# pearl-robot-lab/2HandedAfforder

Hardware: AMD Instinct MI355X
Metric: affordance frames/sec/GPU @1024^2, 32-tok prompt; mask IoU vs ref (higher is better)
Workload: dtype bf16; 1 GPU; BASELINE.json configs[2]: 2HandedAfforder-7B, 64 x 1024x1024 uint8 NHWC frames/step/GPU, 32-token prompt (T=291), 8 forced answer tokens with [SEG], KV-cached greedy decode, random-init weights; CLIP + SAM preprocessing of the uint8 frames on the device inside the step; parallelism=frame-sharded replicas x1 (no collective), hip_streams=2, fp32_decoder_tail=True, fp32_residual_stream=off, neck_f32=False, sam_chunk=16, sam_waits_for_prefill=False, decode_chain=False

## Files before the change

2handedafforder_amd/csrc/gemm_f32.hip:

```cpp
#include "haff_common.h"

namespace {

constexpr int TM = 128, TN = 128, TK = 16, RS = 20;

struct GemmF32Args {
  const float* A; long lda;
  const float* W; long ldw;
  float* C; long ldc;
  const float* bias;
  const float* resid; long ldr;
  const int* row_map;
  int M, N, K;
  int act, swiglu;
  int nb_inner;
  long sAo, sAi, sWo, sWi, sCo, sCi;
};

__global__ __launch_bounds__(256) void gemm_f32_kernel(GemmF32Args p) {
  __shared__ __attribute__((aligned(16))) float sA[2][TM * RS];
  __shared__ __attribute__((aligned(16))) float sW[2][TN * RS];
  if (p.nb_inner > 0) {
    const int zo = blockIdx.y / p.nb_inner, zi = blockIdx.y - zo * p.nb_inner;
    p.A += zo * p.sAo + zi * p.sAi;
    p.W += zo * p.sWo + zi * p.sWi;
    p.C += zo * p.sCo + zi * p.sCi;
  }
  const int tid = threadIdx.x, lane = tid & 63, wave = tid >> 6;
  const int wm = wave & 1, wn = wave >> 1;
  const int fr = lane & 15, fg = lane >> 4;
  const int tiles_n = (p.N + TN - 1) / TN;
  const int tm = blockIdx.x / tiles_n, tn = blockIdx.x - tm * tiles_n;
  const int m0 = tm * TM, n0 = tn * TN;

  f32x4 acc[4][4];
#pragma unroll
  for (int i = 0; i < 4; ++i)
#pragma unroll
    for (int j = 0; j < 4; ++j) acc[i][j] = f32x4{0.f, 0.f, 0.f, 0.f};

  const int lrow = tid >> 2, lk = (tid & 3) * 4;
  const float* a0 = p.A + (long)min(m0 + lrow, p.M - 1) * p.lda + lk;
  const float* a1 = p.A + (long)min(m0 + lrow + 64, p.M - 1) * p.lda + lk;
  const float* w0 = p.W + (long)min(n0 + lrow, p.N - 1) * p.ldw + lk;
  const float* w1 = p.W + (long)min(n0 + lrow + 64, p.N - 1) * p.ldw + lk;
  const float4 z4 = make_float4(0.f, 0.f, 0.f, 0.f);
  float4 ra0, ra1, rw0, rw1;
  auto fetch = [&](int k0) {
    const bool ok = k0 + lk < p.K;
    ra0 = ok ? *reinterpret_cast<const float4*>(a0 + k0) : z4;
    ra1 = ok ? *reinterpret_cast<const float4*>(a1 + k0) : z4;
    rw0 = ok ? *reinterpret_cast<const float4*>(w0 + k0) : z4;
    rw1 = ok ? *reinterpret_cast<const float4*>(w1 + k0) : z4;
  };
  auto stash = [&](int buf) {
    *reinterpret_cast<float4*>(&sA[buf][lrow * RS + lk]) = ra0;
    *reinterpret_cast<float4*>(&sA[buf][(lrow + 64) * RS + lk]) = ra1;
    *reinterpret_cast<float4*>(&sW[buf][lrow * RS + lk]) = rw0;
    *reinterpret_cast<float4*>(&sW[buf][(lrow + 64) * RS + lk]) = rw1;
  };
  const int nk = (p.K + TK - 1) / TK;
  fetch(0);
  stash(0);
  __syncthreads();
  for (int kt = 0; kt < nk; ++kt) {
    const int buf = kt & 1;
// ... 137 lines not shown

template <int MR>
static void launch_f32_skinny(const GemmF32Args& p, hipStream_t s) {
  if (p.N >= 2048) hipLaunchKernelGGL((gemm_f32_skinny_kernel<MR, 4>), dim3((p.N + 3) / 4), dim3(256), 0, s, p);
  else if (p.N >= 512) hipLaunchKernelGGL((gemm_f32_skinny_kernel<MR, 2>), dim3((p.N + 1) / 2), dim3(256), 0, s, p);
  else hipLaunchKernelGGL((gemm_f32_skinny_kernel<MR, 1>), dim3(p.N), dim3(256), 0, s, p);
}

}

extern "C" int haff_gemm_f32(const float* A, long lda, const float* W, long ldw, float* C, long ldc,
                             const float* bias, const float* resid, long ldr, const int* row_map, int M, int N, int K,
                             int act, int swiglu, void* stream) {
  if (M <= 0 || N <= 0 || K <= 0 || (K & 3) || (lda & 3) || (ldw & 3)) return HAFF_ERR_BAD_ARG;
  if (swiglu && ((N & 31) || resid)) return HAFF_ERR_BAD_ARG;
  GemmF32Args p{A, lda, W, ldw, C, ldc, bias, resid, ldr, row_map, M, N, K, act, swiglu, 0, 0, 0, 0, 0, 0, 0};
  hipStream_t s = reinterpret_cast<hipStream_t>(stream);
  const bool al16 = ((reinterpret_cast<uintptr_t>(A) | reinterpret_cast<uintptr_t>(W)) & 15) == 0;
  if (!swiglu && al16 && (M <= 8 || (M <= 16 && (long)N * K <= (1L << 21)))) {
    if (M <= 1) launch_f32_skinny<1>(p, s);
    else if (M <= 4) launch_f32_skinny<4>(p, s);
    else if (M <= 8) launch_f32_skinny<8>(p, s);
    else launch_f32_skinny<16>(p, s);
    return haff_check_launch();
  }
  const int tiles = ((M + TM - 1) / TM) * ((N + TN - 1) / TN);
  hipLaunchKernelGGL(gemm_f32_kernel, dim3(tiles), dim3(256), 0, s, p);
  return haff_check_launch();
}

extern "C" int haff_gemm_f32_batched(const float* A, long lda, long sAo, long sAi, const float* W, long ldw, long sWo,
                                     long sWi, float* C, long ldc, long sCo, long sCi, int nb_outer, int nb_inner, int M,
                                     int N, int K, void* stream) {
  if (M <= 0 || N <= 0 || K <= 0 || nb_outer <= 0 || nb_inner <= 0) return HAFF_ERR_BAD_ARG;
  if ((K & 3) || (lda & 3) || (ldw & 3) || (sAo & 3) || (sAi & 3) || (sWo & 3) || (sWi & 3)) return HAFF_ERR_BAD_ARG;
  GemmF32Args p{A, lda, W, ldw, C, ldc, nullptr, nullptr, 0, nullptr, M, N, K, 0, 0, nb_inner, sAo, sAi, sWo, sWi, sCo, sCi};
  const int tiles = ((M + TM - 1) / TM) * ((N + TN - 1) / TN);
  hipLaunchKernelGGL(gemm_f32_kernel, dim3(tiles, nb_outer * nb_inner), dim3(256), 0, reinterpret_cast<hipStream_t>(stream), p);
  return haff_check_launch();
}
```

2handedafforder_amd/lib.py:

```python
import ctypes
import os
import subprocess

_HERE = os.path.dirname(os.path.abspath(__file__))
LIB_PATH = os.environ.get("HAFF_LIB_PATH") or os.path.join(_HERE, "lib", "libhaff_hip.so")
CSRC_DIR = os.path.join(_HERE, "csrc")

c_void_p, c_long, c_int, c_float = ctypes.c_void_p, ctypes.c_long, ctypes.c_int, ctypes.c_float

_PROTOS = {
    "haff_gemm_bf16": [c_void_p, c_long, c_void_p, c_long, c_void_p, c_long, c_void_p, c_void_p, c_long, c_void_p,
                       c_int, c_int, c_int, c_int, c_int, c_int, c_void_p],
    "haff_gemm_bf16_cfg": [c_void_p, c_long, c_void_p, c_long, c_void_p, c_long, c_void_p, c_void_p, c_long, c_void_p,
                           c_int, c_int, c_int, c_int, c_int, c_int, c_int, c_void_p],
    "haff_gemm_bf16_ws": [c_void_p, c_long, c_void_p, c_long, c_void_p, c_long, c_void_p, c_void_p, c_long, c_void_p,
                          c_int, c_int, c_int, c_int, c_int, c_int, c_void_p, c_long, c_void_p],
    "haff_gemm_bf16_rms": [c_void_p, c_long, c_void_p, c_long, c_void_p, c_long, c_void_p, c_void_p, c_long, c_int, c_int, c_int,
                           c_int, c_int, c_int, c_void_p, c_int, c_float, c_void_p, c_void_p, c_void_p],
    "haff_gemm_bf16_gather": [c_void_p, c_long, c_void_p, c_long, c_void_p, c_long, c_void_p, c_long, c_void_p, c_void_p,
                              c_long, c_void_p, c_int, c_int, c_int, c_int, c_int, c_int, c_void_p],
    "haff_gemm_bf16_ln": [c_void_p, c_long, c_void_p, c_long, c_void_p, c_long, c_void_p, c_void_p, c_long, c_void_p,
                          c_void_p, c_void_p, c_int, c_int, c_int, c_int, c_int, c_int, c_void_p],
    "haff_gemm_bf16_heads": [c_void_p, c_long, c_void_p, c_long, c_void_p, c_void_p, c_void_p, c_void_p, c_void_p, c_int, c_int, c_int,
                             c_int, c_int, c_long, c_long, c_void_p],
# ... 33 lines not shown
    "haff_decode_chain_bf16": [c_void_p, c_int, c_int, c_int, c_int, c_int, c_void_p, c_void_p, c_void_p, c_void_p, c_void_p, c_void_p,
                               c_void_p, c_void_p, c_float, c_void_p, c_void_p, c_int, c_float, c_void_p, c_int, c_void_p],
    "haff_decode_chain_supported": [c_int, c_int, c_int, c_int, c_int],
    "haff_decode_chain_status": [c_void_p, c_int, c_void_p],
    "haff_decode_chain_sync_words": [c_int, c_int],
    "haff_row_stats": [c_void_p, c_long, c_void_p, c_int, c_int, c_float, c_int, c_int, c_void_p],
    "haff_row_stats_finalize": [c_void_p, c_void_p, c_int, c_int, c_int, c_float, c_void_p],
    "haff_gemm_bf16_qkv_rope": [c_void_p, c_long, c_void_p, c_long, c_void_p, c_long, c_void_p, c_void_p, c_void_p,
                                c_int, c_int, c_int, c_int, c_int, c_int, c_int, c_void_p],
    "haff_gemm_bf16_rowstats": [c_void_p, c_long, c_void_p, c_long, c_void_p, c_long, c_void_p, c_long, c_void_p, c_void_p,
                                c_long, c_int, c_int, c_int, c_void_p, c_void_p],
    "haff_gemm_bf16_rowstats32": [c_void_p, c_long, c_void_p, c_long, c_void_p, c_long, c_void_p, c_long, c_void_p, c_long, c_void_p,
                                  c_int, c_int, c_int, c_void_p, c_void_p],
    "haff_gemm_f32": [c_void_p, c_long, c_void_p, c_long, c_void_p, c_long, c_void_p, c_void_p, c_long, c_void_p,
                      c_int, c_int, c_int, c_int, c_int, c_void_p],
    "haff_attention_bf16": [c_void_p, c_long, c_long, c_long, c_void_p, c_long, c_long, c_long,
                            c_void_p, c_long, c_long, c_long, c_void_p, c_long, c_long, c_long,
                            c_int, c_int, c_int, c_int, c_int, c_float, c_int, c_int, c_void_p, c_void_p, c_int,
                            c_void_p],
    "haff_attention_f16": [c_void_p, c_long, c_long, c_long, c_void_p, c_long, c_long, c_long,
                           c_void_p, c_long, c_long, c_long, c_void_p, c_long, c_long, c_long,
                           c_int, c_int, c_int, c_int, c_int, c_float, c_int, c_int, c_void_p, c_void_p, c_int,
                           c_void_p],
    "haff_attention_f32": [c_void_p, c_long, c_long, c_long, c_void_p, c_long, c_long, c_long,
                           c_void_p, c_long, c_long, c_long, c_void_p, c_long, c_long, c_long,
                           c_int, c_int, c_int, c_int, c_int, c_float, c_int, c_int, c_void_p, c_void_p, c_int,
                           c_void_p],
    "haff_attention_decode_rows_bf16": [c_void_p, c_long, c_long, c_void_p, c_long, c_long, c_long, c_void_p, c_long, c_long, c_long,
                                        c_void_p, c_long, c_long, c_int, c_int, c_int, c_int, c_float, c_void_p, c_void_p],
    "haff_attention_decode_rows_f16": [c_void_p, c_long, c_long, c_void_p, c_long, c_long, c_long, c_void_p, c_long, c_long, c_long,
# ... 205 lines not shown
```

2handedafforder_amd/ops.py:

```python
import ctypes

import torch

from .lib import check, load_library

ACT_NONE, ACT_GELU, ACT_QUICK_GELU, ACT_RELU, ACT_SILU = 0, 1, 2, 3, 4


def _dt(t):
    if t.dtype == torch.bfloat16:
        return 0
    if t.dtype == torch.float32:
        return 1
    if t.dtype == torch.float16:
        return 3
    raise TypeError(f"unsupported dtype {t.dtype}")


def _fn(lib, name, dtype):
    return getattr(lib, name.replace("_bf16", "_f16") if dtype == torch.float16 else name)


def _stream():
    return torch.cuda.current_stream().cuda_stream
# ... 127 lines not shown
    b = None
    if beta is not None or bias is not None:
        b = torch.zeros((w.shape[0],), dtype=torch.float32, device=w.device)
        if bias is not None:
            b += bias.float()
        if beta is not None:
            b += w.float() @ beta.float()
        b = b.contiguous()
    return wf, colsum, b


SPLIT_ROW_TAIL = True


def linear(x, w, bias=None, act=ACT_NONE, resid=None, row_map=None, out=None, out_rows=None, out_dtype=None,
           swiglu=False, tile_cfg=0, a_map=None, ln_stats=None, ln_colsum=None):
    lib = load_library()
    _req(x, "x")
    assert x.dim() == 2 and w.dim() == 2 and x.stride(1) == 1 and w.stride(1) == 1
    M, K = x.shape
    if a_map is not None:
        assert a_map.dtype == torch.int32 and x.dtype in (torch.bfloat16, torch.float16)
        M = a_map.numel()
    N = w.shape[0]
    assert w.shape[1] == K, (x.shape, w.shape)
    n_out = N // 2 if swiglu else N
    if out_dtype is None:
        out_dtype = x.dtype
    if out is None:
        out = torch.empty((out_rows if out_rows is not None else M, n_out), dtype=out_dtype, device=x.device)
    assert out.stride(1) == 1 and out.shape[1] == n_out
    if resid is not None:
        assert resid.dtype == out.dtype and resid.stride(1) == 1
    if bias is not None:
# ... 643 lines not shown
    return out


def upscale_mask(up1, ln_w, ln_b, w2, b2, hyper, n_prompts, h, w, eps=1e-6):
    lib = load_library()
    _req(up1, "up1")
    assert up1.is_contiguous() and up1.shape == (n_prompts * h * w, 256)
    assert hyper.dtype == torch.float32 and hyper.is_contiguous() and hyper.shape == (n_prompts, 32)
    out = torch.empty((n_prompts, 4 * h, 4 * w), dtype=torch.float32, device=up1.device)
    rc = lib.haff_upscale_mask(up1.data_ptr(), ln_w.data_ptr(), ln_b.data_ptr(), w2.data_ptr(), b2.data_ptr(),
                               hyper.data_ptr(), out.data_ptr(), n_prompts, h, w, float(eps), _dt(up1), _stream())
    check(rc, "haff_upscale_mask")
    return out


def resize_bilinear(x, crop_hw, out_hw):
    lib = load_library()
    _req(x, "x")
    assert x.dtype == torch.float32 and x.is_contiguous() and x.dim() == 3
    N, Hs, Ws = x.shape
    out = torch.empty((N, out_hw[0], out_hw[1]), dtype=torch.float32, device=x.device)
    rc = lib.haff_resize_bilinear(x.data_ptr(), out.data_ptr(), N, Hs, Ws, int(crop_hw[0]), int(crop_hw[1]),
                                  int(out_hw[0]), int(out_hw[1]), _stream())
    check(rc, "haff_resize_bilinear")
    return out


def threshold_masks(x, logit_th=0.0):
    lib = load_library()
    _req(x, "x")
# ... 295 lines not shown
```

2handedafforder_amd/sam.py:

```python
import math

import torch

from . import ops

V = "model.visual_model"


def _f32(t, device):
    return t.to(device=device, dtype=torch.float32).contiguous()


class SamEncoderHip:

    def __init__(self, sd, cfg, dtype, device):
        s = self.cfg = cfg
        self.dtype, self.device = dtype, device
        E = V + ".image_encoder"
        C = s.embed_dim
        g = s.grid
        dev = device
        self.hd = C // s.heads
        self.w_patch = sd[E + ".patch_embed.proj.weight"].reshape(C, -1).to(dev, dtype).contiguous()
        self.b_patch = _f32(sd[E + ".patch_embed.proj.bias"], dev)
# ... 238 lines not shown
                "lin1": lin(L + ".mlp.lin1"), "lin2": lin(L + ".mlp.lin2")})
        self.final = attn(T + ".final_attn_token_to_image")
        self.nf = norm(T + ".norm_final_attn")
        w = sd[pfx + ".output_upscaling.0.weight"]
        self.w_up1 = w.permute(2, 3, 1, 0).reshape(4 * (C // 4), C).to(dev, dtype).contiguous()
        self.b_up1 = _f32(sd[pfx + ".output_upscaling.0.bias"].repeat(4), dev)
        self.ln_up = norm(pfx + ".output_upscaling.1")
        w = sd[pfx + ".output_upscaling.3.weight"]
        self.w_up2 = _f32(w.permute(0, 2, 3, 1).reshape(C // 4, 4 * (C // 8)), dev)
        self.b_up2 = _f32(sd[pfx + ".output_upscaling.3.bias"], dev)
        self.hyper = [[lin(f"{pfx}.output_hypernetworks_mlps.{i}.layers.{j}") for j in range(3)] for i in range(4)]
        self.iou_head = [lin(f"{pfx}.iou_prediction_head.layers.{j}") for j in range(3)]
        if taxonomy_on:
            self.tax = [lin(f"{pfx}.taxonomy_embed.layers.{j}") for j in range(3)]

    def _attend(self, w, q_in, k_in, v_in, P, nq, nk, heads=8):
        qp = ops.linear(q_in, *w["q"])
        kp = ops.linear(k_in, *w["k"])
        vp = ops.linear(v_in, *w["v"])
        d = qp.shape[1] // heads
        q = qp.view(P, nq, heads, d).permute(0, 2, 1, 3)
        k = kp.view(P, nk, heads, d).permute(0, 2, 1, 3)
        v = vp.view(P, nk, heads, d).permute(0, 2, 1, 3)
        a = ops.attention(q, k, v, 1.0 / math.sqrt(d))
        return a.view(P * nq, heads * d), w["out"]

    def _mlp3(self, layers, x, last_f32=True):
        x = ops.linear(x, *layers[0], act=ops.ACT_RELU)
        x = ops.linear(x, *layers[1], act=ops.ACT_RELU)
        return ops.linear(x, *layers[2], out_dtype=torch.float32 if last_f32 else None)

    def __call__(self, src, key_pe, text, grid, taps=None):
        P, N, C = src.shape
        nt = 6
        tokens = torch.cat([self.out_tokens.unsqueeze(0).expand(P, -1, -1), text.view(P, 1, C).to(self.dtype)], dim=1)
        tokens = tokens.contiguous().view(P * nt, C)
        queries = tokens
        keys = src.reshape(P * N, C)
        for li, L in enumerate(self.layers):
            if li == 0:
                a, wo = self._attend(L["self"], queries, queries, queries, P, nt, nt)
                queries = ops.linear(a, *wo)
            else:
                q = ops.add_bcast(queries, tokens)
                a, wo = self._attend(L["self"], q, q, queries, P, nt, nt)
                queries = ops.linear(a, *wo, resid=queries)
            queries = ops.layernorm(queries, *L["n1"], 1e-5)
            q = ops.add_bcast(queries, tokens)
            k = ops.add_bcast(keys, key_pe, mod=N)
            a, wo = self._attend(L["t2i"], q, k, keys, P, nt, N)
            queries = ops.layernorm(ops.linear(a, *wo, resid=queries), *L["n2"], 1e-5)
            h = ops.linear(queries, *L["lin1"], act=ops.ACT_RELU)
            queries = ops.layernorm(ops.linear(h, *L["lin2"], resid=queries), *L["n3"], 1e-5)
            q = ops.add_bcast(queries, tokens)
            a, wo = self._attend(L["i2t"], k, q, queries, P, N, nt)
            keys = ops.layernorm(ops.linear(a, *wo, resid=keys), *L["n4"], 1e-5)
            if taps is not None:
                taps[f"layer{li}.queries"] = queries.float().view(P, nt, C).cpu()
                taps[f"layer{li}.keys"] = keys.float().view(P, N, C).cpu()
        q = ops.add_bcast(queries, tokens)
        k = ops.add_bcast(keys, key_pe, mod=N)
        a, wo = self._attend(self.final, q, k, keys, P, nt, N)
        queries = ops.layernorm(ops.linear(a, *wo, resid=queries), *self.nf, 1e-5)
        hs = queries.view(P, nt, C)
        up1 = ops.linear(keys, self.w_up1, bias=self.b_up1)
        hyper0 = self._mlp3(self.hyper[0], hs[:, 1])
        low_res = ops.upscale_mask(up1, self.ln_up[0], self.ln_up[1], self.w_up2, self.b_up2, hyper0, P, grid, grid)
        iou = self._mlp3(self.iou_head, hs[:, 0])[:, 0:1]
        tax = None
        if self.taxonomy_on:
            tax = ops.softmax_rows(self._mlp3(self.tax, hs[:, 1:5].reshape(P, 4 * C)).contiguous())
        return low_res, iou, tax


class SamPromptDecoderHip:

    def __init__(self, sd, cfg, dtype, device):
        self.cfg, self.dtype, self.device = cfg, dtype, device
        P = V + ".prompt_encoder"
        g = cfg.grid
        C = cfg.out_chans
        G = sd[P + ".pe_layer.positional_encoding_gaussian_matrix"].float().cpu()
# ... 42 lines not shown
```

include/haff_hip.h:

```cpp
#ifndef HAFF_HIP_H
#define HAFF_HIP_H

#ifdef __cplusplus
extern "C" {
#endif

int haff_gemm_bf16(const void* A, long lda, const void* W, long ldw, void* C, long ldc, const float* bias,
                   const void* resid, long ldr, const int* row_map, int M, int N, int K, int act, int out_f32,
                   int swiglu, void* stream);
int haff_gemm_bf16_cfg(const void* A, long lda, const void* W, long ldw, void* C, long ldc, const float* bias,
                       const void* resid, long ldr, const int* row_map, int M, int N, int K, int act, int out_f32,
                       int swiglu, int tile_cfg, void* stream);
int haff_gemm_bf16_ws(const void* A, long lda, const void* W, long ldw, void* C, long ldc, const float* bias,
                      const void* resid, long ldr, const int* row_map, int M, int N, int K, int act, int out_f32,
                      int swiglu, void* workspace, long workspace_bytes, void* stream);
int haff_gemm_f16(const void* A, long lda, const void* W, long ldw, void* C, long ldc, const float* bias,
                  const void* resid, long ldr, const int* row_map, int M, int N, int K, int act, int out_f32,
                  int swiglu, void* stream);
int haff_gemm_f16_cfg(const void* A, long lda, const void* W, long ldw, void* C, long ldc, const float* bias,
                      const void* resid, long ldr, const int* row_map, int M, int N, int K, int act, int out_f32,
                      int swiglu, int tile_cfg, void* stream);
int haff_gemm_f16_ws(const void* A, long lda, const void* W, long ldw, void* C, long ldc, const float* bias,
                     const void* resid, long ldr, const int* row_map, int M, int N, int K, int act, int out_f32,
                     int swiglu, void* workspace, long workspace_bytes, void* stream);
// ... 55 lines not shown
                         const float* ln_stats, const float* ln_colsum, int M, int N, int K, int d, int heads, long part_stride,
                         long head_stride, void* stream);
int haff_gemm_stream_cap(void* stream, int cap);
int haff_gemm_bf16_qkv_rope(const void* A, long lda, const void* Wp, long ldw, void* q_out, long ldq, void* kcache,
                            void* vcache, const float* cos_sin, int B, int T, int Tmax, int pos0, int H, int d, int K,
                            void* stream);
int haff_gemm_bf16_rowstats(const void* A, long lda, const int* a_map, long a_rows, const void* W, long ldw, void* C,
                            long ldc, const float* bias, const void* resid, long ldr, int M, int N, int K,
                            float* stat_out, void* stream);
int haff_gemm_bf16_rowstats32(const void* A, long lda, const int* a_map, long a_rows, const void* W, long ldw, float* X32,
                              long ldx, void* C16, long ldc, const float* bias, int M, int N, int K, float* stat_out,
                              void* stream);
int haff_gemm_f32(const float* A, long lda, const float* W, long ldw, float* C, long ldc, const float* bias,
                  const float* resid, long ldr, const int* row_map, int M, int N, int K, int act, int swiglu,
                  void* stream);

int haff_attention_bf16(const void* q, long q_sb, long q_sh, long q_st, const void* k, long k_sb, long k_sh, long k_st,
                        const void* v, long v_sb, long v_sh, long v_st, void* o, long o_sb, long o_sh, long o_st,
                        int B, int H, int Nq, int Nk, int d, float scale, int causal, int q_pos0,
                        const float* relh, const float* relw, int S, void* stream);
int haff_attention_f16(const void* q, long q_sb, long q_sh, long q_st, const void* k, long k_sb, long k_sh, long k_st,
                       const void* v, long v_sb, long v_sh, long v_st, void* o, long o_sb, long o_sh, long o_st,
                       int B, int H, int Nq, int Nk, int d, float scale, int causal, int q_pos0,
                       const float* relh, const float* relw, int S, void* stream);
int haff_attention_f32(const float* q, long q_sb, long q_sh, long q_st, const float* k, long k_sb, long k_sh, long k_st,
                       const float* v, long v_sb, long v_sh, long v_st, float* o, long o_sb, long o_sh, long o_st,
                       int B, int H, int Nq, int Nk, int d, float scale, int causal, int q_pos0,
                       const float* relh, const float* relw, int S, void* stream);

int haff_attention_decode_rows_bf16(const void* q, long q_sb, long q_sh, const void* k, long k_sb, long k_sh, long k_st,
// ... 110 lines not shown
                      int n_img, int Hd, int dtype, void* stream);
int haff_rope_cache(void* qkv, long ld, void* kcache, void* vcache, const float* cos_sin, int B, int Tq, int Hq, int Hkv,
                    int d, int pos0, int Tmax, int dtype, void* stream);
int haff_rope_cache_rows(void* qkv, long ld, void* kcache, void* vcache, const float* cos_sin, int B, int Tq, int Hq,
                         int Hkv, int d, const int* pos0_rows, int Tmax, int dtype, void* stream);
int haff_argmax_rows(const float* x, long ld, long* out, int rows, int V, void* stream);
int haff_decode_book(const long* nxt_raw, const long* forced, long forced_ld, const int* use_forced, int* steps,
                     unsigned char* finished, long* out_ids, long out_ld, const long* lens, const int* t_rows, long* tok,
                     int* pos, int* nk, const void* h1, void* hidden, long hid_sb, long row_bytes, long pad, long eos, int B,
                     void* stream);
int haff_add_bcast(const void* a, const void* b, void* out, long rows, int C, int mod, int dtype, void* stream);
int haff_softmax_rows(const void* x, float* out, int rows, int C, int dtype, void* stream);

int haff_upscale_mask(const void* up1, const float* ln_w, const float* ln_b, const float* w2, const float* b2,
                      const float* hyper, float* out, int n_prompts, int h, int w, float eps, int dtype, void* stream);
int haff_resize_bilinear(const float* in, float* out, int N, int Hs, int Ws, int Hc, int Wc, int Ho, int Wo,
                         void* stream);
int haff_resample_u8(const void* in, void* out, int B, int Hin, int Win, int Hout, int Wout, int axis, const int* bounds,
                     const int* coeffs, int ksize, void* stream);
int haff_clip_normalize_u8(const void* in, void* out, int B, int Hin, int Win, int top, int left, int S, const float* lut,
                           int out_dtype, void* stream);
int haff_fill_contours_u8(const int* pts, const int* poly_off, const int* poly_plane, const int* desc_dev, int n_poly, int n_planes,
                          void* out, int H, int W, void* stream);
int haff_jitter_stats_u8(const void* frames, int B, int H, int W, const int* flags, const float* factors, void* sums, void* stream);
int haff_augment_u8(const void* in, void* out, int B, int H, int W, const int* flags, const float* factors, const void* sums,
                    void* stream);
int haff_flip_planes_u8(const void* in, void* out, int P, int H, int W, const int* flags, void* stream);
int haff_threshold_masks(const float* in, void* out, long total, float logit_th, void* stream);
int haff_gate_threshold_masks(const float* logits, void* planes, long total, long plane_stride,
                              const float* thresholds_host, int n_th, int on_value, const float* taxonomy, int blank_class,
// ... 91 lines not shown
```

Baseline: 111.8 frames/s.

## Fuse SAM decoder fp32 tail: i2t attention update, upscale-mask, and key-PE add

Adds fused fp32 kernels for the SAM mask decoder. One kernel does the image-to-token attention step in a single pass: Q projection with the positional embedding added, softmax over up to 16 tokens, output projection, residual and layernorm. A second kernel takes the keys through the first upscale projection, layernorm, GELU, the second upscale, the hypernetwork dot product and the pixel-shuffle write. The fp32 GEMM also gains an optional broadcast add on its A operand, so key+PE is never materialised. The aim is to cut the launches and the large intermediate writes and reads of the per-pixel key tensors. The cost is specialised code hardcoded to C=256 with 8 heads, and the fallbacks still depend on those shapes.

```diff
diff --git a/2handedafforder_amd/csrc/decoder_tail.hip b/2handedafforder_amd/csrc/decoder_tail.hip
--- /dev/null
+++ b/2handedafforder_amd/csrc/decoder_tail.hip
@@ -0,0 +1,373 @@
+#include "haff_common.h"
+
+namespace {
+
+constexpr int DC = 256;
+constexpr int DI = 128;
+constexpr int HEADS = 8;
+constexpr int MAXK = 16;
+constexpr int TR = 64;
+constexpr int RS = 20;
+
+struct I2tArgs {
+  const float* x;
+  const float* pe;
+  const float* wq;
+  const float* bq;
+  const float* kp;
+  const float* vp;
+  const float* wo;
+  const float* bo;
+  const float* ln_w;
+  const float* ln_b;
+  float* y;
+  int N, nk;
+  float scale, eps;
+};
+
+__device__ __forceinline__ f32x4 mfma4(const float4 w, const float4 a, f32x4 acc) {
+  acc = __builtin_amdgcn_mfma_f32_16x16x4f32(w.x, a.x, acc, 0, 0, 0);
+  acc = __builtin_amdgcn_mfma_f32_16x16x4f32(w.y, a.y, acc, 0, 0, 0);
+  acc = __builtin_amdgcn_mfma_f32_16x16x4f32(w.z, a.z, acc, 0, 0, 0);
+  acc = __builtin_amdgcn_mfma_f32_16x16x4f32(w.w, a.w, acc, 0, 0, 0);
+  return acc;
+}
+
+template <int T>
+__device__ __forceinline__ float lane_group_sum(float (&t)[T]) {
+#pragma unroll
+  for (int s = T / 2; s >= 1; s >>= 1)
+#pragma unroll
+    for (int i = 0; i < s; ++i) t[i] += t[i + s];
+  float v = t[0];
+  v += __shfl_xor(v, 16);
+  v += __shfl_xor(v, 32);
+  return v;
+}
+
+__global__ __launch_bounds__(256, 2) void i2t_update_f32_kernel(I2tArgs p) {
+  __shared__ __attribute__((aligned(16))) float sW[2][DC * RS];
+  __shared__ __attribute__((aligned(16))) float sK[MAXK * DI];
+  __shared__ __attribute__((aligned(16))) float sV[MAXK * DI];
+  const int tid = threadIdx.x, lane = tid & 63, wave = tid >> 6;
+  const int fr = lane & 15, fg = lane >> 4;
+  const int prompt = blockIdx.y;
+  const int n = blockIdx.x * TR + wave * 16 + fr;
+  const bool live = n < p.N;
+  const int nc = min(n, p.N - 1);
+  const long row = (long)prompt * p.N + nc;
+
+  float4 xf[DC / 16];
+  {
+    const float* xr = p.x + row * DC + fg * 4;
+#pragma unroll
+    for (int t = 0; t < DC / 16; ++t) xf[t] = *reinterpret_cast<const float4*>(xr + t * 16);
+  }
+  for (int i = tid; i < p.nk * (DI / 4); i += 256) {
+    reinterpret_cast<float4*>(sK)[i] = reinterpret_cast<const float4*>(p.kp + (long)prompt * p.nk * DI)[i];
+    reinterpret_cast<float4*>(sV)[i] = reinterpret_cast<const float4*>(p.vp + (long)prompt * p.nk * DI)[i];
+  }
+
+  const int lrow = tid >> 2, lk = (tid & 3) * 4;
+
+  f32x4 q[HEADS];
+#pragma unroll
+  for (int i = 0; i < HEADS; ++i) q[i] = f32x4{0.f, 0.f, 0.f, 0.f};
+  {
+    const float* w0 = p.wq + (long)lrow * DC + lk;
+    const float* w1 = w0 + 64 * DC;
+    const float* per = p.pe + (long)nc * DC + fg * 4;
+    float4 rw0 = *reinterpret_cast<const float4*>(w0), rw1 = *reinterpret_cast<const float4*>(w1);
+    float4 pf = *reinterpret_cast<const float4*>(per);
+    *reinterpret_cast<float4*>(&sW[0][lrow * RS + lk]) = rw0;
+    *reinterpret_cast<float4*>(&sW[0][(lrow + 64) * RS + lk]) = rw1;
+    __syncthreads();
+#pragma unroll
+    for (int kt = 0; kt < DC / 16; ++kt) {
+      const int buf = kt & 1;
+      const float4 pe4 = pf;
+      if (kt + 1 < DC / 16) {
+        rw0 = *reinterpret_cast<const float4*>(w0 + (kt + 1) * 16);
+        rw1 = *reinterpret_cast<const float4*>(w1 + (kt + 1) * 16);
+        pf = *reinterpret_cast<const float4*>(per + (kt + 1) * 16);
+      }
+      const float4 a = make_float4(xf[kt].x + pe4.x, xf[kt].y + pe4.y, xf[kt].z + pe4.z, xf[kt].w + pe4.w);
+#pragma unroll
+      for (int i = 0; i < HEADS; ++i) {
+        const float4 wf = *reinterpret_cast<const float4*>(&sW[buf][(i * 16 + fr) * RS + fg * 4]);
+        q[i] = mfma4(wf, a, q[i]);
+      }
+      if (kt + 1 < DC / 16) {
+        *reinterpret_cast<float4*>(&sW[buf ^ 1][lrow * RS + lk]) = rw0;
+        *reinterpret_cast<float4*>(&sW[buf ^ 1][(lrow + 64) * RS + lk]) = rw1;
+        __syncthreads();
+      }
+    }
+  }
+
+  const float* v0 = p.wo + (long)lrow * DI + lk;
+  float4 ro[4];
+#pragma unroll
+  for (int s = 0; s < 4; ++s) ro[s] = *reinterpret_cast<const float4*>(v0 + (long)s * 64 * DI);
+
+  const int nk = p.nk;
+#pragma unroll
+  for (int h = 0; h < HEADS; ++h) {
+    const float4 b = *reinterpret_cast<const float4*>(p.bq + h * 16 + fg * 4);
+    const float q0 = q[h][0] + b.x, q1 = q[h][1] + b.y, q2 = q[h][2] + b.z, q3 = q[h][3] + b.w;
+    float sc[MAXK];
+    float m = -INFINITY;
+#pragma unroll
+    for (int j = 0; j < MAXK; ++j) {
+      float s = 0.f;
+      if (j < nk) {
+        const float4 kk = *reinterpret_cast<const float4*>(&sK[j * DI + h * 16 + fg * 4]);
+        s = fmaf(q3, kk.w, fmaf(q2, kk.z, fmaf(q1, kk.y, q0 * kk.x)));
+        s += __shfl_xor(s, 16);
+        s += __shfl_xor(s, 32);
+        s *= p.scale;
+        m = fmaxf(m, s);
+      }
+      sc[j] = s;
+    }
+    float sum = 0.f;
+#pragma unroll
+    for (int j = 0; j < MAXK; ++j) {
+      sc[j] = j < nk ? expf(sc[j] - m) : 0.f;
+      sum += sc[j];
+    }
+    const float inv = 1.0f / sum;
+    float o0 = 0.f, o1 = 0.f, o2 = 0.f, o3 = 0.f;
+#pragma unroll
+    for (int j = 0; j < MAXK; ++j) {
+      if (j < nk) {
+        const float pj = sc[j] * inv;
+        const float4 vv = *reinterpret_cast<const float4*>(&sV[j * DI + h * 16 + fg * 4]);
+        o0 = fmaf(pj, vv.x, o0); o1 = fmaf(pj, vv.y, o1); o2 = fmaf(pj, vv.z, o2); o3 = fmaf(pj, vv.w, o3);
+      }
+    }
+    q[h] = f32x4{o0, o1, o2, o3};
+  }
+
+  f32x4 acc[DC / 16];
+#pragma unroll
+  for (int i = 0; i < DC / 16; ++i) acc[i] = f32x4{0.f, 0.f, 0.f, 0.f};
+#pragma unroll
+  for (int s = 0; s < 4; ++s) *reinterpret_cast<float4*>(&sW[0][(lrow + 64 * s) * RS + lk]) = ro[s];
+  __syncthreads();
+#pragma unroll
+  for (int kt = 0; kt < DI / 16; ++kt) {
+    const int buf = kt & 1;
+    if (kt + 1 < DI / 16) {
+#pragma unroll
+      for (int s = 0; s < 4; ++s) ro[s] = *reinterpret_cast<const float4*>(v0 + (long)s * 64 * DI + (kt + 1) * 16);
+    }
+    const float4 a = make_float4(q[kt][0], q[kt][1], q[kt][2], q[kt][3]);
+#pragma unroll
+    for (int i = 0; i < DC / 16; ++i) {
+      const float4 wf = *reinterpret_cast<const float4*>(&sW[buf][(i * 16 + fr) * RS + fg * 4]);
+      acc[i] = mfma4(wf, a, acc[i]);
+    }
+    if (kt + 1 < DI / 16) {
+#pragma unroll
+      for (int s = 0; s < 4; ++s) *reinterpret_cast<float4*>(&sW[buf ^ 1][(lrow + 64 * s) * RS + lk]) = ro[s];
+      __syncthreads();
+    }
+  }
+
+  float ts[DC / 16];
+#pragma unroll
+  for (int i = 0; i < DC / 16; ++i) {
+    const float4 b = *reinterpret_cast<const float4*>(p.bo + i * 16 + fg * 4);
+    acc[i][0] += b.x; acc[i][1] += b.y; acc[i][2] += b.z; acc[i][3] += b.w;
+    acc[i][0] += xf[i].x; acc[i][1] += xf[i].y; acc[i][2] += xf[i].z; acc[i][3] += xf[i].w;
+    ts[i] = (acc[i][0] + acc[i][1]) + (acc[i][2] + acc[i][3]);
+  }
+  const float mean = lane_group_sum<DC / 16>(ts) / (float)DC;
+#pragma unroll
+  for (int i = 0; i < DC / 16; ++i) {
+    const float d0 = acc[i][0] - mean, d1 = acc[i][1] - mean, d2 = acc[i][2] - mean, d3 = acc[i][3] - mean;
+    ts[i] = (d0 * d0 + d1 * d1) + (d2 * d2 + d3 * d3);
+  }
+  const float rstd = 1.0f / sqrtf(lane_group_sum<DC / 16>(ts) / (float)DC + p.eps);
+  if (!live) return;
+  float* yr = p.y + row * DC + fg * 4;
+#pragma unroll
+  for (int i = 0; i < DC / 16; ++i) {
+    const float4 g = *reinterpret_cast<const float4*>(p.ln_w + i * 16 + fg * 4);
+    const float4 b = *reinterpret_cast<const float4*>(p.ln_b + i * 16 + fg * 4);
+    *reinterpret_cast<float4*>(yr + i * 16) =
+        make_float4((acc[i][0] - mean) * rstd * g.x + b.x, (acc[i][1] - mean) * rstd * g.y + b.y,
+                    (acc[i][2] - mean) * rstd * g.z + b.z, (acc[i][3] - mean) * rstd * g.w + b.w);
+  }
+}
+
+constexpr int C1 = 64, C2 = 32;
+constexpr int W2S = C1 + 4;
+
+struct UpKeysArgs {
+  const float* keys;
+  const float* w1;
+  const float* b1;
+  const float* ln_w;
+  const float* ln_b;
+  const float* w2;
+  const float* b2;
+  const float* hyper;
+  float* out;
+  long rows;
+  int h, w;
+  float eps;
+};
+
+__device__ __forceinline__ float gelu_erf(float x) { return 0.5f * x * (1.0f + erff(x * 0.70710678118654752440f)); }
+
+__global__ __launch_bounds__(256, 2) void upscale_mask_keys_f32_kernel(UpKeysArgs p) {
+  __shared__ __attribute__((aligned(16))) float sW[2][C1 * RS];
+  __shared__ __attribute__((aligned(16))) float sW2[4 * C2 * W2S];
+  const int tid = threadIdx.x, lane = tid & 63, wave = tid >> 6;
+  const int fr = lane & 15, fg = lane >> 4;
+  const long m = (long)blockIdx.x * TR + wave * 16 + fr;
+  const bool live = m < p.rows;
+  const long mc = live ? m : p.rows - 1;
+  const long hw = (long)p.h * p.w;
+  const int pr = (int)(mc / hw);
+  const int pix = (int)(mc - pr * hw);
+  const int py = pix / p.w, px = pix - py * p.w;
+
+  float4 xf[DC / 16];
+  {
+    const float* xr = p.keys + mc * DC + fg * 4;
+#pragma unroll
+    for (int t = 0; t < DC / 16; ++t) xf[t] = *reinterpret_cast<const float4*>(xr + t * 16);
+  }
+  for (int i = tid; i < C1 * 4 * C2; i += 256) {
+    const int co = i >> 7, n = i & 127;
+    sW2[n * W2S + co] = p.w2[i];
+  }
+
+  const int lrow = tid >> 2, lk = (tid & 3) * 4;
+  const float* hy = p.hyper + (long)pr * C2;
+  float4 o = make_float4(0.f, 0.f, 0.f, 0.f);
+#pragma unroll 1
+  for (int tap1 = 0; tap1 < 4; ++tap1) {
+    f32x4 acc[C1 / 16];
+#pragma unroll
+    for (int i = 0; i < C1 / 16; ++i) acc[i] = f32x4{0.f, 0.f, 0.f, 0.f};
+    const float* w0 = p.w1 + (long)(tap1 * C1 + lrow) * DC + lk;
+    float4 rw = *reinterpret_cast<const float4*>(w0);
+    *reinterpret_cast<float4*>(&sW[0][lrow * RS + lk]) = rw;
+    __syncthreads();
+#pragma unroll
+    for (int kt = 0; kt < DC / 16; ++kt) {
+      const int buf = kt & 1;
+      if (kt + 1 < DC / 16) rw = *reinterpret_cast<const float4*>(w0 + (kt + 1) * 16);
+#pragma unroll
+      for (int i = 0; i < C1 / 16; ++i) {
+        const float4 wf = *reinterpret_cast<const float4*>(&sW[buf][(i * 16 + fr) * RS + fg * 4]);
+        acc[i] = mfma4(wf, xf[kt], acc[i]);
+      }
+      if (kt + 1 < DC / 16) {
+        *reinterpret_cast<float4*>(&sW[buf ^ 1][lrow * RS + lk]) = rw;
+        __syncthreads();
+      }
+    }
+    float ts[C1 / 16];
+#pragma unroll
+    for (int i = 0; i < C1 / 16; ++i) {
+      const float4 b = *reinterpret_cast<const float4*>(p.b1 + tap1 * C1 + i * 16 + fg * 4);
+      acc[i][0] += b.x; acc[i][1] += b.y; acc[i][2] += b.z; acc[i][3] += b.w;
+      ts[i] = (acc[i][0] + acc[i][1]) + (acc[i][2] + acc[i][3]);
+    }
+    const float mean = lane_group_sum<C1 / 16>(ts) * (1.0f / C1);
+#pragma unroll
+    for (int i = 0; i < C1 / 16; ++i) {
+      const float d0 = acc[i][0] - mean, d1 = acc[i][1] - mean, d2 = acc[i][2] - mean, d3 = acc[i][3] - mean;
+      ts[i] = (d0 * d0 + d1 * d1) + (d2 * d2 + d3 * d3);
+    }
+    const float rstd = 1.0f / sqrtf(lane_group_sum<C1 / 16>(ts) * (1.0f / C1) + p.eps);
+    float4 vf[C1 / 16];
+#pragma unroll
+    for (int i = 0; i < C1 / 16; ++i) {
+      const float4 g = *reinterpret_cast<const float4*>(p.ln_w + i * 16 + fg * 4);
+      const float4 b = *reinterpret_cast<const float4*>(p.ln_b + i * 16 + fg * 4);
+      vf[i] = make_float4(gelu_erf((acc[i][0] - mean) * rstd * g.x + b.x), gelu_erf((acc[i][1] - mean) * rstd * g.y + b.y),
+                          gelu_erf((acc[i][2] - mean) * rstd * g.z + b.z), gelu_erf((acc[i][3] - mean) * rstd * g.w + b.w));
+    }
+    f32x4 u[4 * C2 / 16];
+#pragma unroll
+    for (int i = 0; i < 4 * C2 / 16; ++i) u[i] = f32x4{0.f, 0.f, 0.f, 0.f};
+#pragma unroll
+    for (int kt = 0; kt < C1 / 16; ++kt)
+#pragma unroll
+      for (int i = 0; i < 4 * C2 / 16; ++i) {
+        const float4 wf = *reinterpret_cast<const float4*>(&sW2[(i * 16 + fr) * W2S + kt * 16 + fg * 4]);
+        u[i] = mfma4(wf, vf[kt], u[i]);
+      }
+    float mt[4];
+#pragma unroll
+    for (int tap2 = 0; tap2 < 4; ++tap2) {
+      float part = 0.f;
+#pragma unroll
+      for (int s = 0; s < 2; ++s) {
+        const int c2 = s * 16 + fg * 4;
+        const float4 b = *reinterpret_cast<const float4*>(p.b2 + c2);
+        const float4 hv = *reinterpret_cast<const float4*>(hy + c2);
+        const f32x4 t = u[tap2 * 2 + s];
+        part += hv.x * gelu_erf(t[0] + b.x);
+        part += hv.y * gelu_erf(t[1] + b.y);
+        part += hv.z * gelu_erf(t[2] + b.z);
+        part += hv.w * gelu_erf(t[3] + b.w);
+      }
+      part += __shfl_xor(part, 16);
+      part += __shfl_xor(part, 32);
+      mt[tap2] = part;
+    }
+    if ((tap1 >> 1) == (fg >> 1)) {
+      const float a = (fg & 1) ? mt[2] : mt[0], b = (fg & 1) ? mt[3] : mt[1];
+      if (tap1 & 1) { o.z = a; o.w = b; } else { o.x = a; o.y = b; }
+    }
+  }
+  if (live) {
+    const long W4 = 4L * p.w;
+    *reinterpret_cast<float4*>(p.out + (long)pr * (4 * p.h) * W4 + (long)(4 * py + fg) * W4 + 4 * px) = o;
+  }
+}
+
+}
+
+extern "C" int haff_upscale_mask_keys_f32(const float* keys, const float* w_up1, const float* b_up1, const float* ln_w,
+                                          const float* ln_b, const float* w2, const float* b2, const float* hyper, float* out,
+                                          int n_prompts, int h, int w, int C, float eps, void* stream) {
+  if (n_prompts <= 0 || h <= 0 || w <= 0 || C <= 0) return HAFF_ERR_BAD_ARG;
+  if (!keys || !w_up1 || !b_up1 || !ln_w || !ln_b || !w2 || !b2 || !hyper || !out) return HAFF_ERR_BAD_ARG;
+  if (C != DC) return HAFF_ERR_UNSUPPORTED;
+  const uintptr_t all = reinterpret_cast<uintptr_t>(keys) | reinterpret_cast<uintptr_t>(w_up1) | reinterpret_cast<uintptr_t>(b_up1) |
+                        reinterpret_cast<uintptr_t>(ln_w) | reinterpret_cast<uintptr_t>(ln_b) | reinterpret_cast<uintptr_t>(w2) |
+                        reinterpret_cast<uintptr_t>(b2) | reinterpret_cast<uintptr_t>(hyper) | reinterpret_cast<uintptr_t>(out);
+  if (all & 15) return HAFF_ERR_UNSUPPORTED;
+  const long rows = (long)n_prompts * h * w;
+  if ((rows + TR - 1) / TR > 0x7fffffffL) return HAFF_ERR_UNSUPPORTED;
+  UpKeysArgs p{keys, w_up1, b_up1, ln_w, ln_b, w2, b2, hyper, out, rows, h, w, eps};
+  hipLaunchKernelGGL(upscale_mask_keys_f32_kernel, dim3((unsigned)((rows + TR - 1) / TR)), dim3(256), 0,
+                     reinterpret_cast<hipStream_t>(stream), p);
+  return haff_check_launch();
+}
+
+extern "C" int haff_i2t_update_f32(const float* x, const float* pe, const float* wq, const float* bq, const float* kp,
+                                   const float* vp, const float* wo, const float* bo, const float* ln_w, const float* ln_b,
+                                   float* y, int n_prompts, int n_rows, int nk, int C, int internal, int heads, float scale,
+                                   float eps, void* stream) {
+  if (n_prompts <= 0 || n_rows <= 0 || nk <= 0 || C <= 0 || internal <= 0 || heads <= 0) return HAFF_ERR_BAD_ARG;
+  if (!x || !pe || !wq || !bq || !kp || !vp || !wo || !bo || !ln_w || !ln_b || !y) return HAFF_ERR_BAD_ARG;
+  if (C != DC || internal != DI || heads != HEADS || nk > MAXK || n_prompts > 65535) return HAFF_ERR_UNSUPPORTED;
+  const uintptr_t all = reinterpret_cast<uintptr_t>(x) | reinterpret_cast<uintptr_t>(pe) | reinterpret_cast<uintptr_t>(wq) |
+                        reinterpret_cast<uintptr_t>(bq) | reinterpret_cast<uintptr_t>(kp) | reinterpret_cast<uintptr_t>(vp) |
+                        reinterpret_cast<uintptr_t>(wo) | reinterpret_cast<uintptr_t>(bo) | reinterpret_cast<uintptr_t>(ln_w) |
+                        reinterpret_cast<uintptr_t>(ln_b) | reinterpret_cast<uintptr_t>(y);
+  if (all & 15) return HAFF_ERR_UNSUPPORTED;
+  I2tArgs p{x, pe, wq, bq, kp, vp, wo, bo, ln_w, ln_b, y, n_rows, nk, scale, eps};
+  dim3 g((n_rows + TR - 1) / TR, n_prompts);
+  hipLaunchKernelGGL(i2t_update_f32_kernel, g, dim3(256), 0, reinterpret_cast<hipStream_t>(stream), p);
+  return haff_check_launch();
+}
diff --git a/2handedafforder_amd/csrc/gemm_f32.hip b/2handedafforder_amd/csrc/gemm_f32.hip
--- a/2handedafforder_amd/csrc/gemm_f32.hip
+++ b/2handedafforder_amd/csrc/gemm_f32.hip
@@ -15,6 +15,7 @@
   int act, swiglu;
   int nb_inner;
   long sAo, sAi, sWo, sWi, sCo, sCi;
+  const float* a_add; int a_add_mod;
 };
 
 __global__ __launch_bounds__(256) void gemm_f32_kernel(GemmF32Args p) {
@@ -44,12 +45,19 @@
   const float* a1 = p.A + (long)min(m0 + lrow + 64, p.M - 1) * p.lda + lk;
   const float* w0 = p.W + (long)min(n0 + lrow, p.N - 1) * p.ldw + lk;
   const float* w1 = p.W + (long)min(n0 + lrow + 64, p.N - 1) * p.ldw + lk;
+  const float* d0 = p.a_add ? p.a_add + (long)(min(m0 + lrow, p.M - 1) % p.a_add_mod) * p.K + lk : nullptr;
+  const float* d1 = p.a_add ? p.a_add + (long)(min(m0 + lrow + 64, p.M - 1) % p.a_add_mod) * p.K + lk : nullptr;
   const float4 z4 = make_float4(0.f, 0.f, 0.f, 0.f);
   float4 ra0, ra1, rw0, rw1;
   auto fetch = [&](int k0) {
     const bool ok = k0 + lk < p.K;
     ra0 = ok ? *reinterpret_cast<const float4*>(a0 + k0) : z4;
     ra1 = ok ? *reinterpret_cast<const float4*>(a1 + k0) : z4;
+    if (p.a_add && ok) {
+      const float4 e0 = *reinterpret_cast<const float4*>(d0 + k0), e1 = *reinterpret_cast<const float4*>(d1 + k0);
+      ra0.x += e0.x; ra0.y += e0.y; ra0.z += e0.z; ra0.w += e0.w;
+      ra1.x += e1.x; ra1.y += e1.y; ra1.z += e1.z; ra1.w += e1.w;
+    }
     rw0 = ok ? *reinterpret_cast<const float4*>(w0 + k0) : z4;
     rw1 = ok ? *reinterpret_cast<const float4*>(w1 + k0) : z4;
   };
@@ -217,7 +225,7 @@
                              int act, int swiglu, void* stream) {
   if (M <= 0 || N <= 0 || K <= 0 || (K & 3) || (lda & 3) || (ldw & 3)) return HAFF_ERR_BAD_ARG;
   if (swiglu && ((N & 31) || resid)) return HAFF_ERR_BAD_ARG;
-  GemmF32Args p{A, lda, W, ldw, C, ldc, bias, resid, ldr, row_map, M, N, K, act, swiglu, 0, 0, 0, 0, 0, 0, 0};
+  GemmF32Args p{A, lda, W, ldw, C, ldc, bias, resid, ldr, row_map, M, N, K, act, swiglu, 0, 0, 0, 0, 0, 0, 0, nullptr, 0};
   hipStream_t s = reinterpret_cast<hipStream_t>(stream);
   const bool al16 = ((reinterpret_cast<uintptr_t>(A) | reinterpret_cast<uintptr_t>(W)) & 15) == 0;
   if (!swiglu && al16 && (M <= 8 || (M <= 16 && (long)N * K <= (1L << 21)))) {
@@ -232,12 +240,23 @@
   return haff_check_launch();
 }
 
+extern "C" int haff_gemm_f32_aadd(const float* A, long lda, const float* a_add, int a_add_mod, const float* W, long ldw, float* C,
+                                  long ldc, const float* bias, const float* resid, long ldr, int M, int N, int K, int act,
+                                  void* stream) {
+  if (M <= 0 || N <= 0 || K <= 0 || (K & 3) || (lda & 3) || (ldw & 3) || !a_add || a_add_mod <= 0) return HAFF_ERR_BAD_ARG;
+  if (M <= 16 || (reinterpret_cast<uintptr_t>(a_add) & 15)) return HAFF_ERR_UNSUPPORTED;
+  GemmF32Args p{A, lda, W, ldw, C, ldc, bias, resid, ldr, nullptr, M, N, K, act, 0, 0, 0, 0, 0, 0, 0, 0, a_add, a_add_mod};
+  const int tiles = ((M + TM - 1) / TM) * ((N + TN - 1) / TN);
+  hipLaunchKernelGGL(gemm_f32_kernel, dim3(tiles), dim3(256), 0, reinterpret_cast<hipStream_t>(stream), p);
+  return haff_check_launch();
+}
+
 extern "C" int haff_gemm_f32_batched(const float* A, long lda, long sAo, long sAi, const float* W, long ldw, long sWo,
                                      long sWi, float* C, long ldc, long sCo, long sCi, int nb_outer, int nb_inner, int M,
                                      int N, int K, void* stream) {
   if (M <= 0 || N <= 0 || K <= 0 || nb_outer <= 0 || nb_inner <= 0) return HAFF_ERR_BAD_ARG;
   if ((K & 3) || (lda & 3) || (ldw & 3) || (sAo & 3) || (sAi & 3) || (sWo & 3) || (sWi & 3)) return HAFF_ERR_BAD_ARG;
-  GemmF32Args p{A, lda, W, ldw, C, ldc, nullptr, nullptr, 0, nullptr, M, N, K, 0, 0, nb_inner, sAo, sAi, sWo, sWi, sCo, sCi};
+  GemmF32Args p{A, lda, W, ldw, C, ldc, nullptr, nullptr, 0, nullptr, M, N, K, 0, 0, nb_inner, sAo, sAi, sWo, sWi, sCo, sCi, nullptr, 0};
   const int tiles = ((M + TM - 1) / TM) * ((N + TN - 1) / TN);
   hipLaunchKernelGGL(gemm_f32_kernel, dim3(tiles, nb_outer * nb_inner), dim3(256), 0, reinterpret_cast<hipStream_t>(stream), p);
   return haff_check_launch();
diff --git a/2handedafforder_amd/lib.py b/2handedafforder_amd/lib.py
--- a/2handedafforder_amd/lib.py
+++ b/2handedafforder_amd/lib.py
@@ -71,6 +71,12 @@
                                   c_int, c_int, c_int, c_void_p, c_void_p],
     "haff_gemm_f32": [c_void_p, c_long, c_void_p, c_long, c_void_p, c_long, c_void_p, c_void_p, c_long, c_void_p,
                       c_int, c_int, c_int, c_int, c_int, c_void_p],
+    "haff_gemm_f32_aadd": [c_void_p, c_long, c_void_p, c_int, c_void_p, c_long, c_void_p, c_long, c_void_p, c_void_p, c_long,
+                           c_int, c_int, c_int, c_int, c_void_p],
+    "haff_upscale_mask_keys_f32": [c_void_p, c_void_p, c_void_p, c_void_p, c_void_p, c_void_p, c_void_p, c_void_p, c_void_p,
+                                   c_int, c_int, c_int, c_int, c_float, c_void_p],
+    "haff_i2t_update_f32": [c_void_p, c_void_p, c_void_p, c_void_p, c_void_p, c_void_p, c_void_p, c_void_p, c_void_p, c_void_p,
+                            c_void_p, c_int, c_int, c_int, c_int, c_int, c_int, c_float, c_float, c_void_p],
     "haff_attention_bf16": [c_void_p, c_long, c_long, c_long, c_void_p, c_long, c_long, c_long,
                             c_void_p, c_long, c_long, c_long, c_void_p, c_long, c_long, c_long,
                             c_int, c_int, c_int, c_int, c_int, c_float, c_int, c_int, c_void_p, c_void_p, c_int,
diff --git a/2handedafforder_amd/ops.py b/2handedafforder_amd/ops.py
--- a/2handedafforder_amd/ops.py
+++ b/2handedafforder_amd/ops.py
@@ -165,10 +165,33 @@
 
 
 def linear(x, w, bias=None, act=ACT_NONE, resid=None, row_map=None, out=None, out_rows=None, out_dtype=None,
-           swiglu=False, tile_cfg=0, a_map=None, ln_stats=None, ln_colsum=None):
+           swiglu=False, tile_cfg=0, a_map=None, ln_stats=None, ln_colsum=None, a_add=None, a_add_mod=None):
     lib = load_library()
     _req(x, "x")
     assert x.dim() == 2 and w.dim() == 2 and x.stride(1) == 1 and w.stride(1) == 1
+    if a_add is not None:
+        assert a_map is None and ln_stats is None and row_map is None and not swiglu and a_add.dtype == x.dtype and a_add.is_contiguous()
+        mod = a_add.shape[0] if a_add_mod is None else int(a_add_mod)
+        assert a_add.shape == (mod, x.shape[1])
+        if x.dtype == torch.float32 and w.dtype == torch.float32 and out_dtype in (None, torch.float32) and out_rows is None:
+            M, K = x.shape
+            N = w.shape[0]
+            assert w.shape[1] == K, (x.shape, w.shape)
+            y = torch.empty((M, N), dtype=torch.float32, device=x.device) if out is None else out
+            assert y.dtype == torch.float32 and y.shape == (M, N) and y.stride(1) == 1
+            if resid is not None:
+                assert resid.dtype == torch.float32 and resid.stride(1) == 1
+            if bias is not None:
+                assert bias.dtype == torch.float32 and bias.numel() == N
+            rc = lib.haff_gemm_f32_aadd(x.data_ptr(), x.stride(0), a_add.data_ptr(), mod, w.data_ptr(), w.stride(0), y.data_ptr(),
+                                        y.stride(0), _p(bias), _p(resid), 0 if resid is None else resid.stride(0), M, N, K, act,
+                                        _stream())
+            if rc == 0:
+                return y
+            if rc != -2:
+                check(rc, "haff_gemm_f32_aadd")
+            out = y
+        x = add_bcast(x.contiguous(), a_add, mod)
     M, K = x.shape
     if a_map is not None:
         assert a_map.dtype == torch.int32 and x.dtype in (torch.bfloat16, torch.float16)
@@ -842,6 +865,49 @@
     return out
 
 
+def upscale_mask_keys(keys, w_up1, b_up1, ln_w, ln_b, w2, b2, hyper, n_prompts, h, w, eps=1e-6):
+    lib = load_library()
+    _req(keys, "keys")
+    ts = (keys, w_up1, b_up1, ln_w, ln_b, w2, b2, hyper)
+    if any(t.dtype != torch.float32 or not t.is_contiguous() for t in ts):
+        return None
+    C = keys.shape[1]
+    if C != 256:
+        return None
+    assert keys.shape == (n_prompts * h * w, C) and w_up1.shape == (256, C) and b_up1.numel() == 256 and w2.shape == (64, 128)
+    assert hyper.shape == (n_prompts, 32) and ln_w.numel() == 64 and ln_b.numel() == 64 and b2.numel() == 32
+    out = torch.empty((n_prompts, 4 * h, 4 * w), dtype=torch.float32, device=keys.device)
+    rc = lib.haff_upscale_mask_keys_f32(keys.data_ptr(), w_up1.data_ptr(), b_up1.data_ptr(), ln_w.data_ptr(), ln_b.data_ptr(),
+                                        w2.data_ptr(), b2.data_ptr(), hyper.data_ptr(), out.data_ptr(), n_prompts, h, w, C,
+                                        float(eps), _stream())
+    if rc == -2:
+        return None
+    check(rc, "haff_upscale_mask_keys_f32")
+    return out
+
+
+def i2t_update(x, pe, wq, bq, kp, vp, wo, bo, ln_w, ln_b, n_prompts, heads=8, eps=1e-5):
+    lib = load_library()
+    _req(x, "x")
+    ts = (x, pe, wq, bq, kp, vp, wo, bo, ln_w, ln_b)
+    if any(t.dtype != torch.float32 or not t.is_contiguous() for t in ts):
+        return None
+    R, C = x.shape
+    N, Ci = pe.shape[0], wq.shape[0]
+    nk = kp.shape[0] // n_prompts
+    assert R == n_prompts * N and pe.shape == (N, C) and wq.shape == (Ci, C) and wo.shape == (C, Ci) and Ci % heads == 0
+    assert kp.shape == (n_prompts * nk, Ci) and vp.shape == kp.shape and bq.numel() == Ci
+    assert bo.numel() == C and ln_w.numel() == C and ln_b.numel() == C
+    out = torch.empty_like(x)
+    rc = lib.haff_i2t_update_f32(x.data_ptr(), pe.data_ptr(), wq.data_ptr(), bq.data_ptr(), kp.data_ptr(), vp.data_ptr(),
+                                 wo.data_ptr(), bo.data_ptr(), ln_w.data_ptr(), ln_b.data_ptr(), out.data_ptr(), n_prompts, N, nk,
+                                 C, Ci, heads, 1.0 / (Ci // heads) ** 0.5, float(eps), _stream())
+    if rc == -2:
+        return None
+    check(rc, "haff_i2t_update_f32")
+    return out
+
+
 def resize_bilinear(x, crop_hw, out_hw):
     lib = load_library()
     _req(x, "x")
diff --git a/2handedafforder_amd/sam.py b/2handedafforder_amd/sam.py
--- a/2handedafforder_amd/sam.py
+++ b/2handedafforder_amd/sam.py
@@ -276,9 +276,11 @@
         if taxonomy_on:
             self.tax = [lin(f"{pfx}.taxonomy_embed.layers.{j}") for j in range(3)]
 
-    def _attend(self, w, q_in, k_in, v_in, P, nq, nk, heads=8):
+    fused_tail = True
+
+    def _attend(self, w, q_in, k_in, v_in, P, nq, nk, heads=8, k_add=None):
         qp = ops.linear(q_in, *w["q"])
-        kp = ops.linear(k_in, *w["k"])
+        kp = ops.linear(k_in, *w["k"], a_add=k_add)
         vp = ops.linear(v_in, *w["v"])
         d = qp.shape[1] // heads
         q = qp.view(P, nq, heads, d).permute(0, 2, 1, 3)
@@ -299,6 +301,7 @@
         tokens = tokens.contiguous().view(P * nt, C)
         queries = tokens
         keys = src.reshape(P * N, C)
+        fused = self.fused_tail and self.dtype == torch.float32
         for li, L in enumerate(self.layers):
             if li == 0:
                 a, wo = self._attend(L["self"], queries, queries, queries, P, nt, nt)
@@ -309,25 +312,45 @@
                 queries = ops.linear(a, *wo, resid=queries)
             queries = ops.layernorm(queries, *L["n1"], 1e-5)
             q = ops.add_bcast(queries, tokens)
-            k = ops.add_bcast(keys, key_pe, mod=N)
-            a, wo = self._attend(L["t2i"], q, k, keys, P, nt, N)
+            if fused:
+                k = None
+                a, wo = self._attend(L["t2i"], q, keys, keys, P, nt, N, k_add=key_pe)
+            else:
+                k = ops.add_bcast(keys, key_pe, mod=N)
+                a, wo = self._attend(L["t2i"], q, k, keys, P, nt, N)
             queries = ops.layernorm(ops.linear(a, *wo, resid=queries), *L["n2"], 1e-5)
             h = ops.linear(queries, *L["lin1"], act=ops.ACT_RELU)
             queries = ops.layernorm(ops.linear(h, *L["lin2"], resid=queries), *L["n3"], 1e-5)
             q = ops.add_bcast(queries, tokens)
-            a, wo = self._attend(L["i2t"], k, q, queries, P, N, nt)
-            keys = ops.layernorm(ops.linear(a, *wo, resid=keys), *L["n4"], 1e-5)
+            new_keys = None
+            if fused:
+                w = L["i2t"]
+                new_keys = ops.i2t_update(keys, key_pe, *w["q"], ops.linear(q, *w["k"]), ops.linear(queries, *w["v"]), *w["out"],
+                                          *L["n4"], P)
+            if new_keys is None:
+                if k is None:
+                    k = ops.add_bcast(keys, key_pe, mod=N)
+                a, wo = self._attend(L["i2t"], k, q, queries, P, N, nt)
+                new_keys = ops.layernorm(ops.linear(a, *wo, resid=keys), *L["n4"], 1e-5)
+            keys = new_keys
             if taps is not None:
                 taps[f"layer{li}.queries"] = queries.float().view(P, nt, C).cpu()
                 taps[f"layer{li}.keys"] = keys.float().view(P, N, C).cpu()
         q = ops.add_bcast(queries, tokens)
-        k = ops.add_bcast(keys, key_pe, mod=N)
-        a, wo = self._attend(self.final, q, k, keys, P, nt, N)
+        if fused:
+            a, wo = self._attend(self.final, q, keys, keys, P, nt, N, k_add=key_pe)
+        else:
+            a, wo = self._attend(self.final, q, ops.add_bcast(keys, key_pe, mod=N), keys, P, nt, N)
         queries = ops.layernorm(ops.linear(a, *wo, resid=queries), *self.nf, 1e-5)
         hs = queries.view(P, nt, C)
-        up1 = ops.linear(keys, self.w_up1, bias=self.b_up1)
         hyper0 = self._mlp3(self.hyper[0], hs[:, 1])
-        low_res = ops.upscale_mask(up1, self.ln_up[0], self.ln_up[1], self.w_up2, self.b_up2, hyper0, P, grid, grid)
+        low_res = None
+        if fused:
+            low_res = ops.upscale_mask_keys(keys, self.w_up1, self.b_up1, self.ln_up[0], self.ln_up[1], self.w_up2, self.b_up2,
+                                            hyper0, P, grid, grid)
+        if low_res is None:
+            up1 = ops.linear(keys, self.w_up1, bias=self.b_up1)
+            low_res = ops.upscale_mask(up1, self.ln_up[0], self.ln_up[1], self.w_up2, self.b_up2, hyper0, P, grid, grid)
         iou = self._mlp3(self.iou_head, hs[:, 0])[:, 0:1]
         tax = None
         if self.taxonomy_on:
diff --git a/include/haff_hip.h b/include/haff_hip.h
--- a/include/haff_hip.h
+++ b/include/haff_hip.h
@@ -93,6 +93,8 @@
 int haff_gemm_f32(const float* A, long lda, const float* W, long ldw, float* C, long ldc, const float* bias,
                   const float* resid, long ldr, const int* row_map, int M, int N, int K, int act, int swiglu,
                   void* stream);
+int haff_gemm_f32_aadd(const float* A, long lda, const float* a_add, int a_add_mod, const float* W, long ldw, float* C, long ldc,
+                       const float* bias, const float* resid, long ldr, int M, int N, int K, int act, void* stream);
 
 int haff_attention_bf16(const void* q, long q_sb, long q_sh, long q_st, const void* k, long k_sb, long k_sh, long k_st,
                         const void* v, long v_sb, long v_sh, long v_st, void* o, long o_sb, long o_sh, long o_st,
@@ -233,6 +235,12 @@
 
 int haff_upscale_mask(const void* up1, const float* ln_w, const float* ln_b, const float* w2, const float* b2,
                       const float* hyper, float* out, int n_prompts, int h, int w, float eps, int dtype, void* stream);
+int haff_upscale_mask_keys_f32(const float* keys, const float* w_up1, const float* b_up1, const float* ln_w, const float* ln_b,
+                               const float* w2, const float* b2, const float* hyper, float* out, int n_prompts, int h, int w,
+                               int C, float eps, void* stream);
+int haff_i2t_update_f32(const float* x, const float* pe, const float* wq, const float* bq, const float* kp, const float* vp,
+                        const float* wo, const float* bo, const float* ln_w, const float* ln_b, float* y, int n_prompts,
+                        int n_rows, int nk, int C, int internal, int heads, float scale, float eps, void* stream);
 int haff_resize_bilinear(const float* in, float* out, int N, int Hs, int Ws, int Hc, int Wc, int Ho, int Wo,
                          void* stream);
 int haff_resample_u8(const void* in, void* out, int B, int Hin, int Win, int Hout, int Wout, int axis, const int* bounds,
```

Result: no change. 112.0 frames/s (median of 6 runs) (+0.2%).
